# jskvrna/MonoSOWA

Hardware: AMD Instinct MI355X
Metric: MonoDETR training img/s (KITTI 1280x384) (higher is better)
Workload: dtype f32; 1 GPU; MonoDETR resnet50 KITTI 1280x384, fwd+criterion+bwd+AdamW step, per-GPU batch 16, synthetic images + random pseudo-labels; global_batch=16, per_gpu_batch=16, parallelism=dp1, accumulation_micro_steps=1, mixed_cameras=False, queries=550, tuned=True

## Files before the change

### monosowa_amd/csrc/msda_capi.hip

```cpp
#include "../../include/monosowa_msda.h"
#include "msda_kernels.hip"
#include "msda_backward_tiled.hip"
#include "msda_backward_sorted.hip"
#include "msda_backward_bands.hip"
#include "msda_gather_rec.hip"
#include "msda_gather_win.hip"
#include "msda_scatter_rows.hip"
#include "msda_plan.hip"
#include <map>
#include <mutex>
#include <cstdlib>
#include <string>
#include <algorithm>
#include <vector>

namespace {

inline int grid_for(long long work_items, int items_per_block) {
  long long g = (work_items + items_per_block - 1) / items_per_block;
  const long long cap = 256LL * 64;
  if (g > cap) g = cap;
  if (g < 1) g = 1;
  return (int)g;
}

inline int grid_pairs(long long n_pairs) { return (int)(((n_pairs + 31) / 32 + 7) / 8 * 8); }

inline int check_dims(int B, int S, int M, int D, int L, int Lq, int P) {
  if (B <= 0 || S <= 0 || M <= 0 || D <= 0 || L <= 0 || Lq <= 0 || P <= 0) return MSDA_E_SHAPE;
  if ((long long)S * M * D >= (1LL << 31)) return MSDA_E_SHAPE;
  if ((long long)B * Lq * M >= (1LL << 35)) return MSDA_E_SHAPE;
  return 0;
}

struct Options {
  int gather = 2;
  int scatter_fixed = 1;
  int scatter_sorted = 0;
  int gather_chunks_fwd = 16, gather_chunks_bwd = 8;
  int window = 3;
  int window_halo = 5;
  int window_persistent = 1;
  int scatter_rows = 1;
  int scatter_reach = 6;
  int directional = 1;
  int scatter_lists = 0;
  int scatter_lists_cap = 0;
  int scatter_bands = 1;
  int plan_fused = 1;
  int plan_reach = 8;
  int deterministic = 0;
  Options() {
    if (const char *e = std::getenv("MSDA_GATHER")) gather = std::atoi(e);
    if (const char *e = std::getenv("MSDA_SCATTER_FIXED")) scatter_fixed = std::atoi(e) != 0;
    if (const char *e = std::getenv("MSDA_SCATTER_SORTED")) scatter_sorted = std::atoi(e);
    if (const char *e = std::getenv("MSDA_GATHER_CHUNKS")) gather_chunks_fwd = std::max(1, std::atoi(e));
    if (const char *e = std::getenv("MSDA_GATHER_CHUNKS_BWD")) gather_chunks_bwd = std::max(1, std::atoi(e));
    if (const char *e = std::getenv("MSDA_WINDOW")) window = std::atoi(e) & 3;
    if (const char *e = std::getenv("MSDA_WINDOW_PERSISTENT")) window_persistent = std::atoi(e) != 0;
    if (const char *e = std::getenv("MSDA_SCATTER_ROWS")) scatter_rows = std::atoi(e) != 0;
    if (const char *e = std::getenv("MSDA_SCATTER_REACH")) scatter_reach = std::min(16, std::max(1, std::atoi(e)));
    if (const char *e = std::getenv("MSDA_WINDOW_HALO")) window_halo = std::min(32, std::max(0, std::atoi(e)));
    if (const char *e = std::getenv("MSDA_DIRECTIONAL")) directional = std::atoi(e) != 0;
    if (const char *e = std::getenv("MSDA_SCATTER_BANDS")) scatter_bands = std::atoi(e) != 0;
    if (const char *e = std::getenv("MSDA_SCATTER_LISTS")) scatter_lists = std::atoi(e) != 0;
    if (const char *e = std::getenv("MSDA_PLAN_FUSED")) plan_fused = std::atoi(e) != 0;
    if (const char *e = std::getenv("MSDA_PLAN_REACH")) plan_reach = std::min(16, std::max(1, std::atoi(e)));
  }
};
inline Options &options() {
  static Options o;
  return o;
}
inline bool scatter_fixed_point() { return options().scatter_fixed != 0; }
inline int gather_mode() { return options().gather; }
inline int gather_chunks_fwd() { return options().gather_chunks_fwd; }
inline int gather_chunks_bwd() { return options().gather_chunks_bwd; }

inline int check_host_geometry(const int64_t *shapes_host, const int64_t *lsi_host, int L, int S) {
  long long next = 0;
  for (int l = 0; l < L; ++l) {
    const long long H = shapes_host[2 * l], W = shapes_host[2 * l + 1];
    if (H <= 0 || W <= 0 || H > 32000 || W > 32000) return MSDA_E_SHAPE;
    if (lsi_host[l] != next) return MSDA_E_SHAPE;
    next += H * W;
  }
  return next == S ? 0 : MSDA_E_SHAPE;
}

bool make_gather_geom(const int64_t *shapes_host, const int64_t *lsi_host, int B, int M, int Lq, int S,
                      msda::GatherGeom &g, bool bwd = false) {
  int first = 4;
  long long rows = 0;
// ... 47 lines not shown
  static std::map<std::vector<int64_t>, msda::WinQuery *> cache;
  int dev = 0;
  if (hipGetDevice(&dev) != hipSuccess) return nullptr;
  std::vector<int64_t> key(shapes_host, shapes_host + 8);
  key.insert(key.end(), lsi_host, lsi_host + 4);
  key.push_back(halo);
  key.push_back(bwd);
  key.push_back(dev);
  std::lock_guard<std::mutex> lock(mu);
  auto it = cache.find(key);
  if (it == cache.end()) {
    std::vector<msda::WinQuery> host((size_t)wt.n_ty * wt.n_tx * msda::kWinMaxQueries * msda::kWinLevels);
    msda::fill_query_table(wt, host.data());
    msda::WinQuery *devp = nullptr;
    if (hipMalloc(&devp, host.size() * sizeof(msda::WinQuery)) != hipSuccess) return nullptr;
    if (hipMemcpy(devp, host.data(), host.size() * sizeof(msda::WinQuery), hipMemcpyHostToDevice) != hipSuccess) {
      (void)hipFree(devp);
      return nullptr;
    }
    it = cache.emplace(key, devp).first;
  }
  return it->second;
}

inline int persistent_grid() {
  static const int n = [] {
    int dev = 0, cus = 256;
    hipDeviceProp_t prop;
    if (hipGetDevice(&dev) == hipSuccess && hipGetDeviceProperties(&prop, dev) == hipSuccess && prop.multiProcessorCount > 0)
      cus = prop.multiProcessorCount;
    return std::max(8, cus / 8 * 8);
  }();
  return n;
}

constexpr int kWinMaxStride = 4096;
inline bool window_fits(int S, long long widest_stride) { return S < (1 << 17) && widest_stride <= kWinMaxStride; }

inline bool window_applies(bool bwd, const int64_t *shapes_host, const int64_t *lsi_host, int Lq, int S, long long widest_stride) {
  msda::WinGeom wg;
  return Lq == S && (options().window & (bwd ? 2 : 1)) && gather_mode() > 1 && window_fits(S, widest_stride) &&
         window_tiling(shapes_host, lsi_host, options().window_halo, bwd, wg);
}

thread_local int tl_launch_error = 0;
inline int launch_status() {
  const int e = tl_launch_error;
  tl_launch_error = 0;
  return e ? e : (int)hipGetLastError();
}

struct ValueView {
  int token_stride = 0;
  const unsigned char *mask = nullptr;
};

template <bool BWD, bool FUSED, bool SAVED = false>
void launch_gather(const float *value, const float *loc, const float *attw, const float *grad_out, float *out,
                   float *grad_loc, float *grad_attw, const float *ref, int ref_dim, const int64_t *shapes_host,
                   const int64_t *lsi_host, int B, int S, int M, int Lq, hipStream_t stream, int loc_rs = 0, int aw_rs = 0,
                   float *grad_value = nullptr, int far_reach = -1, ValueView vv = ValueView(),
                   const msda::HeadPlan *plans = nullptr, const unsigned char *far_mask = nullptr) {
  if (!loc_rs) loc_rs = M * 32;
  if (!aw_rs) aw_rs = M * 16;
  const int vts = vv.token_stride ? vv.token_stride : M * 32;
  if (Lq == S && (options().window & (BWD ? 2 : 1)) && gather_mode() > 1 && (!FUSED || ref_dim == 2)) {
// ... 170 lines not shown
            const int tiles = rp.n_ty[l] * rp.n_tx[l];
            bp.cap[l] = (int)std::min<long long>((3LL * Lq + tiles - 1) / tiles + 256, 16LL * msda::kRowChunkQueries);
            if (options().scatter_lists_cap > 0) bp.cap[l] = std::min(bp.cap[l], options().scatter_lists_cap);
            bp.list_off[l] = entries;
            n_tiles += tiles;
            entries += tiles * bp.cap[l];
            rp.n_chunks[l] = std::max(1, std::min(16, (bp.cap[l] + msda::kRowChunkQueries - 1) / msda::kRowChunkQueries));
            work[l] = (double)bp.cap[l] / rp.n_chunks[l];
            rp.order[l] = l;
          }
          bp.n_tiles = n_tiles; bp.plane_entries = entries;
          std::sort(rp.order, rp.order + 4, [&](int a, int b) { return work[a] > work[b]; });
          rp.first_item[0] = 0;
          for (int i = 0; i < 4; ++i) rp.first_item[i + 1] = rp.first_item[i] + rp.n_ty[rp.order[i]] * rp.n_tx[rp.order[i]] * rp.n_chunks[rp.order[i]];
          rp.n_items = rp.first_item[4];
          const size_t counts_b = align256(sizeof(unsigned) * (size_t)B * M * n_tiles);
          const size_t lists_b = align256(sizeof(unsigned) * (size_t)B * M * entries);
          const size_t far_b = align256((size_t)B * M * 4 * S);
          if ((long long)B * M * entries < (1LL << 31) && counts_b + lists_b + far_b <= workspace_bytes) {
            char *wsp = reinterpret_cast<char *>(workspace);
            unsigned *counts = reinterpret_cast<unsigned *>(wsp);
            unsigned *lists = reinterpret_cast<unsigned *>(wsp + counts_b);
            unsigned char *far_mask = reinterpret_cast<unsigned char *>(wsp + counts_b + lists_b);
            hipError_t e = hipMemsetAsync(counts, 0, counts_b, stream);
            if (e != hipSuccess) return (int)e;
            const long long n_units = (long long)B * M * 4 * S;
            msda::bin_points_kernel<<<(unsigned)((n_units + 255) / 256), 256, 0, stream>>>(loc, bp, n_units, S, counts, lists, far_mask);
            for (int l = 0; l < L; ++l) {
              if (rp.n_chunks[l] == 1) continue;
              e = hipMemset2DAsync(grad_value + (size_t)rp.start[l] * M * 32, sizeof(float) * (size_t)S * M * 32, 0,
                                   sizeof(float) * (size_t)rp.H[l] * rp.W[l] * M * 32, B, stream);
              if (e != hipSuccess) return (int)e;
            }
            const int groups = (B * M + 7) / 8;
            msda::scatter_rows_kernel<false, true><<<8 * rp.n_items * groups, msda::kRowThreads, 0, stream>>>(
                loc, attw, grad_out, grad_value, nullptr, 0, nullptr, rp, B, S, M, 0, 0, vv.mask, nullptr, lists, counts, bp, far_mask);
            launch_gather<true, true, true>(value, loc, attw, grad_out, nullptr, grad_loc, grad_attw, fused_ref, fused_ref_dim,
                                            shapes_host, lsi_host, B, S, M, Lq, stream, loc_rs, aw_rs, grad_value, 0, vv, nullptr, far_mask);
            return launch_status();
          }
        }
        bool directional = options().directional && (saved || fused_ref) && M <= msda::kPlanMaxHeads;
        int reach = 0;
        size_t plan_b = 0, stats_b = 0;
        bool ok = false;
        for (int attempt = 0; attempt < 2 && !ok; ++attempt) {
          reach = directional ? std::max(options().scatter_reach, options().plan_reach) : options().scatter_reach;
          plan_b = directional ? align256(msda::plan_bytes(M)) : 0;
          stats_b = directional ? align256(msda::plan_stats_bytes(M) * msda::kStatsBlocks) : 0;
          ok = msda::make_row_plan(shapes_host, lsi_host, reach, rp) && (!directional || rp.n_items <= msda::kPlanMaxItems) &&
               plan_b + stats_b + msda::row_plan_table_bytes(rp) * (directional ? M : 1) <= workspace_bytes;
          if (!ok) { if (!directional) break; directional = false; }
        }
        if (ok) {
          char *wsp = reinterpret_cast<char *>(workspace);
          msda::HeadPlan *plans = directional ? reinterpret_cast<msda::HeadPlan *>(wsp) : nullptr;
          msda::RowCandidate *table = reinterpret_cast<msda::RowCandidate *>(wsp + plan_b + stats_b);
          int n_tiles = 0;
          for (int l = 0; l < 4; ++l) n_tiles += rp.n_ty[l] * rp.n_tx[l];
          if (plan_mode && !(directional && saved)) return MSDA_E_UNSUPPORTED;
          if (directional && plan_mode != 2) {
            msda::PlanGeom pg{};
            for (int l = 0; l < 4; ++l) { pg.H[l] = rp.H[l]; pg.W[l] = rp.W[l]; pg.start[l] = rp.start[l]; }
            pg.S = S; pg.M = M;
            pg.default_halo = options().window_halo;
            pg.reach = reach;
            pg.want_rows = 1;
            if (options().plan_fused) {
              if (saved)
                msda::plan_fused_kernel<1><<<M * n_tiles, 256, 0, stream>>>(loc, nullptr, pg, rp, B, 0, n_tiles, plans, table);
              else
                msda::plan_fused_kernel<0><<<M * n_tiles, 256, 0, stream>>>(loc, fused_ref, pg, rp, B, loc_rs ? loc_rs : M * 32, n_tiles,
                                                                            plans, table);
            } else {
              msda::DirStats *partial = reinterpret_cast<msda::DirStats *>(wsp + plan_b);
              if (saved)
                msda::dir_stats_kernel<1><<<msda::kStatsBlocks, msda::kStatsThreads, 0, stream>>>(loc, nullptr, pg, B, 0, partial);
              else
                msda::dir_stats_kernel<0><<<msda::kStatsBlocks, msda::kStatsThreads, 0, stream>>>(
                    loc, fused_ref, pg, B, loc_rs ? loc_rs : M * 32, partial);
              msda::dir_plan_kernel<<<M, 256, 0, stream>>>(partial, msda::kStatsBlocks, pg, rp, plans);
            }
          }
          if (plan_mode != 2 && !(directional && options().plan_fused))
            msda::row_candidates_kernel<<<n_tiles * (directional ? M : 1), 256, 0, stream>>>(rp, table, plans, n_tiles);
          if (plan_mode == 1) return launch_status();
          for (int l = 0; l < L; ++l) {
            if (rp.n_chunks[l] == 1) continue;
            hipError_t e = hipMemset2DAsync(grad_value + (size_t)rp.start[l] * M * 32, sizeof(float) * (size_t)S * M * 32, 0,
                                            sizeof(float) * (size_t)rp.H[l] * rp.W[l] * M * 32, B, stream);
            if (e != hipSuccess) return (int)e;
          }
          const int groups = (B * M + 7) / 8;
          const int lrs = loc_rs ? loc_rs : M * 32, ars = aw_rs ? aw_rs : M * 16;
          if (fused_ref && !saved)
            msda::scatter_rows_kernel<true><<<8 * rp.n_items * groups, msda::kRowThreads, 0, stream>>>(
                loc, attw, grad_out, grad_value, fused_ref, fused_ref_dim, table, rp, B, S, M, lrs, ars, vv.mask, plans);
          else if (saved)
            msda::scatter_rows_kernel<false, true><<<8 * rp.n_items * groups, msda::kRowThreads, 0, stream>>>(
                loc, attw, grad_out, grad_value, nullptr, 0, table, rp, B, S, M, 0, 0, vv.mask, plans);
          else
            msda::scatter_rows_kernel<false><<<8 * rp.n_items * groups, msda::kRowThreads, 0, stream>>>(
                loc, attw, grad_out, grad_value, nullptr, 0, table, rp, B, S, M, lrs, ars);
          if (fused_ref && saved)
            launch_gather<true, true, true>(value, loc, attw, grad_out, nullptr, grad_loc, grad_attw, fused_ref, fused_ref_dim,
                                            shapes_host, lsi_host, B, S, M, Lq, stream, loc_rs, aw_rs, grad_value, rp.reach, vv, plans);
          else if (fused_ref)
            launch_gather<true, true>(value, loc, attw, grad_out, nullptr, grad_loc, grad_attw, fused_ref, fused_ref_dim,
                                      shapes_host, lsi_host, B, S, M, Lq, stream, loc_rs, aw_rs, grad_value, rp.reach, vv, plans);
          else
            launch_gather<true, false>(value, loc, attw, grad_out, nullptr, grad_loc, grad_attw, nullptr, 0, shapes_host,
                                       lsi_host, B, S, M, Lq, stream, 0, 0, grad_value, rp.reach);
          return launch_status();
        }
      }
      if (saved || plan_mode) return MSDA_E_UNSUPPORTED;
      const msda::BwdPlan plan = make_plan(shapes_host, lsi_host, L, Lq, P, det);
      if ((long long)Lq * P >= (1LL << (62 - msda::kFixBits))) return MSDA_E_SHAPE;
      const TiledWorkspace ws = tiled_workspace(B, M, L, Lq, P);
      char *wsp = reinterpret_cast<char *>(workspace);
      float2 *rec_hw = reinterpret_cast<float2 *>(wsp);
      float *rec_aw = reinterpret_cast<float *>(wsp + ws.off_aw);
      msda::ChunkBox *boxes = reinterpret_cast<msda::ChunkBox *>(wsp + ws.off_boxes);
      float *bounds = reinterpret_cast<float *>(wsp + ws.off_bounds);
      if (fused_ref)
        msda::bwd_prep_kernel<4, true><<<(unsigned)(B * ws.n_chunks_per_list), M * L * 8, 0, stream>>>(
            loc, attw, grad_out, shapes, rec_hw, rec_aw, boxes, fused_ref, fused_ref_dim, M, L, Lq, (int)ws.n_chunks_per_list,
            loc_rs ? loc_rs : M * 32, aw_rs ? aw_rs : M * 16);
      else
        msda::bwd_prep_kernel<4, false><<<(unsigned)(B * ws.n_chunks_per_list), M * L * 8, 0, stream>>>(
            loc, attw, grad_out, shapes, rec_hw, rec_aw, boxes, nullptr, 0, M, L, Lq, (int)ws.n_chunks_per_list, M * 32, M * 16);
      msda::BandPlan bp;
      const bool bands = !det && options().scatter_bands && options().scatter_sorted != 2 && L == 4 && P == 4 &&
                         msda::make_band_plan(shapes_host, lsi_host, Lq, bp);
      if (!bands) msda::bwd_bounds_kernel<<<B * M, 256, 0, stream>>>(boxes, bounds, (int)(L * ws.n_chunks_per_list));
      for (int l = 0; l < L && !bands; ++l) {
// ... 24 lines not shown
          launch_gather<true, false>(value, loc, attw, grad_out, nullptr, grad_loc, grad_attw, nullptr, 0, shapes_host,
                                     lsi_host, B, S, M, Lq, stream);
      } else {
        msda::bwd_gather_kernel<4, 4><<<grid_pairs(n_pairs), 256, 0, stream>>>(
            value, shapes, lsi, loc, attw, grad_out, grad_loc, grad_attw, S, M, Lq, n_pairs);
      }
      return launch_status();
    }
  }
  hipError_t err = hipMemsetAsync(grad_value, 0, sizeof(T) * (size_t)B * S * M * D, stream);
  if (err != hipSuccess) return (int)err;
  msda::bwd_generic_kernel<T><<<grid_for(n_pairs, 8), 256, 0, stream>>>(
      value, shapes, lsi, loc, attw, grad_out, grad_value, grad_loc, grad_attw, S, M, D, L, Lq, P,
      n_pairs);
  return launch_status();
}

}

extern "C" {

int msda_abi_version(void) { return MSDA_ABI_VERSION; }

int msda_set_option(const char *name, int value) {
  if (!name) return MSDA_E_NULLPTR;
  const std::string n(name);
  if (n == "gather" && value >= 0 && value <= 2) { options().gather = value; return 0; }
  if (n == "scatter_fixed" && (value == 0 || value == 1)) { options().scatter_fixed = value; return 0; }
  if (n == "scatter_sorted" && value >= 0 && value <= 2) { options().scatter_sorted = value; return 0; }
  if (n == "window" && value >= 0 && value <= 3) { options().window = value; return 0; }
  if (n == "window_halo" && value >= 0 && value <= 32) { options().window_halo = value; return 0; }
  if (n == "window_persistent" && (value == 0 || value == 1)) { options().window_persistent = value; return 0; }
  if (n == "scatter_rows" && (value == 0 || value == 1)) { options().scatter_rows = value; return 0; }
  if (n == "scatter_reach" && value >= 1 && value <= 16) { options().scatter_reach = value; return 0; }
  if (n == "directional" && (value == 0 || value == 1)) { options().directional = value; return 0; }
  if (n == "scatter_bands" && (value == 0 || value == 1)) { options().scatter_bands = value; return 0; }
  if (n == "scatter_lists" && (value == 0 || value == 1)) { options().scatter_lists = value; return 0; }
  if (n == "plan_reach" && value >= 1 && value <= 16) { options().plan_reach = value; return 0; }
  if (n == "plan_fused" && (value == 0 || value == 1)) { options().plan_fused = value; return 0; }
  if (n == "scatter_lists_cap" && value >= 0) { options().scatter_lists_cap = value; return 0; }
  if (n == "deterministic" && (value == 0 || value == 1)) { options().deterministic = value; return 0; }
  return MSDA_E_UNSUPPORTED;
}

int msda_options_stamp(void) {
  const Options &o = options();
  unsigned h = 2166136261u;
  for (int v : {o.directional, o.scatter_lists, o.scatter_rows, o.scatter_reach, o.plan_reach, o.plan_fused, o.window, o.window_halo, o.gather, o.deterministic}) {
    h ^= (unsigned)v + 0x9E3779B9u;
    h *= 16777619u;
  }
  return (int)(h & 0x7FFFFFFFu);
}

int msda_debug_counter(const char *name, unsigned long long *out) {
  if (!name || !out) return MSDA_E_NULLPTR;
  const std::string n(name);
  static const char *const scan_names[5] = {"scan_candidates", "scan_delivering", "scan_point_tests", "scan_delivered", "scan_points_skipped"};
  int scan = -1;
  for (int i = 0; i < 5; ++i)
    if (n == scan_names[i]) scan = i;
  if (n != "scatter_overflow_rounds" && scan < 0) return MSDA_E_UNSUPPORTED;
  const unsigned long long zero = 0;
  hipError_t e = hipDeviceSynchronize();
  if (scan >= 0) {
    if (e == hipSuccess) e = hipMemcpyFromSymbol(out, HIP_SYMBOL(msda::g_rows_scan), sizeof(zero), scan * sizeof(zero));
    if (e == hipSuccess) e = hipMemcpyToSymbol(HIP_SYMBOL(msda::g_rows_scan), &zero, sizeof(zero), scan * sizeof(zero));
    return (int)e;
  }
  if (e == hipSuccess) e = hipMemcpyFromSymbol(out, HIP_SYMBOL(msda::g_rows_overflow_rounds), sizeof(zero));
  if (e == hipSuccess) e = hipMemcpyToSymbol(HIP_SYMBOL(msda::g_rows_overflow_rounds), &zero, sizeof(zero));
  return (int)e;
}

const char *msda_strerror(int code) {
  switch (code) {
    case 0: return "success";
    case MSDA_E_NULLPTR: return "msda: a required pointer is NULL";
    case MSDA_E_SHAPE: return "msda: a dimension is <= 0 or exceeds the indexing range";
    case MSDA_E_UNSUPPORTED: return "msda: unsupported configuration";
    case MSDA_E_WORKSPACE: return "msda: workspace is NULL or smaller than msda_backward_workspace_bytes()";
// ... 261 lines not shown
```

### monosowa_amd/csrc/msda_scatter_rows.hip

```cpp
#include "msda_common.h"
#include "msda_scatter_plan.h"
#include "msda_plan.h"
#include "msda_bin.hip"

#ifndef MSDA_ROWS_SKIP
#define MSDA_ROWS_SKIP 0
#endif
#ifndef MSDA_ROWS_STAMP
#define MSDA_ROWS_STAMP 0
#endif

namespace msda {

#if MSDA_ROWS_STAMP
__device__ unsigned long long g_rows_stamp[8];
#define ROWS_STAMP(i) do { const long long t_ = clock64(); st_acc[i] += t_ - st_t; st_t = t_; } while (0)
#else
#define ROWS_STAMP(i) do { } while (0)
#endif

typedef float rows_v2f __attribute__((ext_vector_type(2)));

__device__ unsigned long long g_rows_overflow_rounds;

#ifndef MSDA_ROWS_PRIO
#define MSDA_ROWS_PRIO 0
#endif
#ifndef MSDA_ROWS_COUNT
#define MSDA_ROWS_COUNT 0
#endif
__device__ unsigned long long g_rows_scan[5];

__device__ __forceinline__ void lds_barrier() {
  asm volatile("s_waitcnt lgkmcnt(0)\n\ts_barrier" ::: "memory");
}

__global__ __launch_bounds__(256) void row_candidates_kernel(const RowPlan p, RowCandidate *__restrict__ table,
                                                             const HeadPlan *__restrict__ plans, int n_tiles) {
  const int head = blockIdx.x / n_tiles;
  int l = 0, t = blockIdx.x - head * n_tiles;
  while (l < 3 && t >= p.n_ty[l] * p.n_tx[l]) { t -= p.n_ty[l] * p.n_tx[l]; ++l; }
  const int ty = t / p.n_tx[l], tx = t - ty * p.n_tx[l];
  const RowAxis *axes = plans ? plans[head].rax : p.ax;
  const RowAxis ay = axes[p.axis0[l] + ty], ax = axes[p.axis0[l] + p.n_ty[l] + tx];
  RowCandidate *out = table + (long long)head * p.cand_total + p.cand_base[l] + (long long)t * p.cand_stride[l];
  int first = 0;
  for (int lq = 0; lq < 4; ++lq) {
    const int n = (int)ay.qn[lq] * (int)ax.qn[lq], w = ax.qn[lq];
    for (int k = threadIdx.x; k < n; k += 256) {
      const int dy = k / w, dx = k - dy * w;
      const int yq = ay.q0[lq] + dy, xq = ax.q0[lq] + dx;
      RowCandidate c;
      c.token = p.start[lq] + yq * p.W[lq] + xq;
      c.cy = (short)centre_floor(yq, p.H[lq], p.H[l]);
      c.cx = (short)centre_floor(xq, p.W[lq], p.W[l]);
      out[first + k] = c;
    }
    first += n;
  }
}

#ifndef MSDA_ROW_WAVES
#define MSDA_ROW_WAVES 4
#endif
template <bool FUSED, bool LEVEL_MAJOR = false>
__global__ __launch_bounds__(kRowThreads, MSDA_ROW_WAVES) void scatter_rows_kernel(
    const float *__restrict__ loc, const float *__restrict__ attw, const float *__restrict__ grad_out,
    float *__restrict__ grad_value, const float *__restrict__ ref, int ref_dim, const RowCandidate *__restrict__ table,
    const RowPlan p, int B, int S, int M, int loc_rs, int aw_rs, const unsigned char *__restrict__ vmask = nullptr,
    const HeadPlan *__restrict__ plans = nullptr, const unsigned *__restrict__ lists = nullptr,
    const unsigned *__restrict__ counts = nullptr, const BinPlan bp = BinPlan(),
    const unsigned char *__restrict__ far_mask = nullptr) {
  __shared__ float4 lds_pool[kRowBatchQueries * 8 + kRowBatchQueries * 4];
  float4 *const go_lds = lds_pool;
  float4 *const coef_tab = lds_pool + kRowBatchQueries * 8;
  static_assert(kRowThreads * 6 <= kRowBatchQueries * 12, "the epilogue's exchange fits the pool");
  __shared__ unsigned short bucket[kRowTileRows * (kRowCellCap + 1)];
  __shared__ unsigned count[kRowTileRows];
  __shared__ int overflow;

  const int bm = (int)(blockIdx.x % 8) + 8 * (int)(blockIdx.x / (8 * p.n_items));
  if (bm >= B * M) return;
  const int it = (int)((blockIdx.x / 8) % p.n_items);
  const int b = bm / M, m = bm - b * M;
  const HeadPlan *hp = plans ? plans + m : nullptr;
  int l, n_chunks, y0, th, x0, tw, c_begin, c_end;
  const RowCandidate *cands;
  DirBounds nb;
  bool by_list = false;
  const unsigned *list = nullptr;
  if (lists) {
    int oi = 0;
    while (oi < 3 && it >= p.first_item[oi + 1]) ++oi;
    l = p.order[oi];
    const int local = it - p.first_item[oi];
    n_chunks = p.n_chunks[l];
    const int chunk = local % n_chunks, tile = local / n_chunks;
    const int ty = tile / p.n_tx[l], tx = tile - ty * p.n_tx[l];
    const RowAxis ay = p.ax[p.axis0[l] + ty], ax = p.ax[p.axis0[l] + p.n_ty[l] + tx];
    y0 = ay.r0; x0 = ax.r0; th = ay.rn; tw = ax.rn;
    const int n_list = (int)min(counts[(long long)bm * bp.n_tiles + bp.tile0[l] + tile], (unsigned)bp.cap[l]);
    c_begin = chunk * kRowChunkQueries;
    c_end = min(n_list, c_begin + kRowChunkQueries);
    if (c_end <= c_begin) {
      if (chunk > 0) return;
      c_end = c_begin;
    }
    list = lists + (long long)bm * bp.plane_entries + bp.list_off[l] + (long long)tile * bp.cap[l];
    cands = nullptr;
    nb.ylo = nb.xlo = nb.yhi = nb.xhi = 0;
    by_list = true;
  } else if (hp) {
    if (it >= hp->n_items) return;
    const RowItem d = hp->items[it];
    l = d.level; n_chunks = d.n_chunks;
    y0 = d.y0; th = d.th; x0 = d.x0; tw = d.tw;
    c_begin = d.c_begin; c_end = d.c_end;
    cands = table + (long long)m * p.cand_total + d.cand_off;
    nb = d.near;
  } else {
    int oi = 0;
    while (oi < 3 && it >= p.first_item[oi + 1]) ++oi;
    l = p.order[oi];
    const int local = it - p.first_item[oi];
    n_chunks = p.n_chunks[l];
    const int chunk = local % n_chunks, tile = local / n_chunks;
    const int ty = tile / p.n_tx[l], tx = tile - ty * p.n_tx[l];
    const RowAxis ay = p.ax[p.axis0[l] + ty], ax = p.ax[p.axis0[l] + p.n_ty[l] + tx];
    nb.ylo = nb.xlo = (short)-p.reach; nb.yhi = nb.xhi = (short)p.reach;
    y0 = ay.r0; x0 = ax.r0; th = ay.rn; tw = ax.rn;
    int n_cand = 0;
#pragma unroll
    for (int lq = 0; lq < 4; ++lq) n_cand += (int)ay.qn[lq] * (int)ax.qn[lq];
    c_begin = (int)((long long)n_cand * chunk / n_chunks);
    c_end = (int)((long long)n_cand * (chunk + 1) / n_chunks);
    cands = table + p.cand_base[l] + (long long)tile * p.cand_stride[l];
  }
  const int H = p.H[l], W = p.W[l];
  const int cw = tw + 1, n_cells = (th + 1) * cw;
  constexpr int cap = kRowCellCap, bstride = kRowCellCap + 1;

  const int tid = threadIdx.x;
  const int slot0 = tid >> 2, pt = tid & 3;
  const int cell = tid >> 2, quarter = tid & 3;
  if (tid < kRowTileRows) count[tid] = 0;
  if (tid == 0) overflow = 0;
  rows_v2f sums[4][4];
#pragma unroll
  for (int j = 0; j < 4; ++j)
#pragma unroll
    for (int i = 0; i < 4; ++i) sums[j][i] = (rows_v2f){0.f, 0.f};

  struct Points { float4 lg; float2 xy; float wt; RefScale rs; };
  const int n_batches = (MSDA_ROWS_SKIP & 128) ? 1 : (c_end - c_begin + kRowBatchQueries - 1) / kRowBatchQueries;
  auto cand_index = [&](const int k, const int u) {
    return k < n_batches ? c_begin + k + (slot0 + u * (kRowThreads / 4)) * n_batches : c_end;
  };
  auto candidate = [&](const int j) {
    RowCandidate c{-1, 0, 0};
    if (j < c_end) {
      if (by_list) {
        const unsigned e = list[j];
        c.token = (int)(e & 0x0FFFFFFFu);
        c.cy = (short)((e >> 28) & ~(unsigned)far_mask[((long long)bm * 4 + l) * S + c.token]);
      } else {
        c = cands[j];
      }
    }
    return c;
  };
#if MSDA_ROWS_COUNT
  unsigned n_scan[5] = {0, 0, 0, 0, 0};
#endif
  auto fetch = [&](const RowCandidate c) {
    Points in{};
    if (c.token >= 0) {
      const long long q_lin = (long long)b * S + c.token;
      const long long pl = (((long long)(b * M + m) * 4 + l) * S + c.token) * 4 + pt;
      in.xy = LEVEL_MAJOR ? *reinterpret_cast<const float2 *>(loc + pl * 2)
                          : *reinterpret_cast<const float2 *>(loc + q_lin * loc_rs + ((m * 4 + l) * 4 + pt) * 2);
      if (FUSED) {
        const float *lg = attw + q_lin * aw_rs + m * 16;
        in.lg = ld4(lg + pt * 4);
        in.wt = lg[l * 4 + pt];
        in.rs = load_ref(ref + (q_lin * 4 + l) * ref_dim, ref_dim, H, W);
      } else {
        in.wt = LEVEL_MAJOR ? attw[pl] : attw[q_lin * aw_rs + (m * 4 + l) * 4 + pt];
      }
    }
    return in;
  };
  RowCandidate cur[kRowSub], c_next[kRowSub];
  Points in[kRowSub];
#pragma unroll
  for (int u = 0; u < kRowSub; ++u) {
    cur[u] = candidate(cand_index(0, u));
    in[u] = fetch(cur[u]);
    c_next[u] = candidate(cand_index(1, u));
  }
  lds_barrier();
#if MSDA_ROWS_STAMP
  long long st_acc[8] = {0, 0, 0, 0, 0, 0, 0, 0}, st_t = clock64();
#endif

  for (int k = 0; k < n_batches; ++k) {
    ROWS_STAMP(0);
#if MSDA_ROWS_PRIO == 1
    __builtin_amdgcn_s_setprio(2);
#elif MSDA_ROWS_PRIO == 2
    __builtin_amdgcn_s_setprio(0);
#endif
    float4 g0[kRowSub], g1[kRowSub];
#pragma unroll
    for (int u = 0; u < kRowSub; ++u) {
      g0[u] = g1[u] = make_float4(0.f, 0.f, 0.f, 0.f);
      if (cur[u].token >= 0 && !(MSDA_ROWS_SKIP & 16)) {
        const float *gp = grad_out + (((long long)b * S + cur[u].token) * M + m) * 32 + pt * 8;
        g0[u] = ld4(gp);
        g1[u] = ld4(gp + 4);
      }
    }
    unsigned pend = 0;
    int cells[kRowSub];
#pragma unroll
    for (int u = 0; u < kRowSub; ++u) {
      const int slot = slot0 + u * (kRowThreads / 4);
      float lx = in[u].xy.x, ly = in[u].xy.y, wt = in[u].wt;
      if (FUSED) {
        const float4 lg = in[u].lg;
        float mx = fmaxf(fmaxf(lg.x, lg.y), fmaxf(lg.z, lg.w));
        mx = fmaxf(mx, dpp_x<0xB1>(mx)); mx = fmaxf(mx, dpp_x<0x4E>(mx));
        float sum = expf(lg.x - mx) + expf(lg.y - mx) + expf(lg.z - mx) + expf(lg.w - mx);
        sum += dpp_x<0xB1>(sum); sum += dpp_x<0x4E>(sum);
        wt = expf(wt - mx) / sum;
        lx = loc_from_offset<4>(in[u].rs.rx, lx, in[u].rs.sx, ref_dim);
        ly = loc_from_offset<4>(in[u].rs.ry, ly, in[u].rs.sy, ref_dim);
      }
      cells[u] = 0;
      if (cur[u].token >= 0 && (!(MSDA_ROWS_SKIP & 32) || lx == 123.456f)) {
#if MSDA_ROWS_COUNT
        n_scan[0] += pt == 0;
        ++n_scan[2];
#endif
        const Tap<float> tp = make_tap<float>(lx, ly, H, W);
        if (tp.valid && (by_list ? (cur[u].cy >> pt & 1) != 0 : inside_bounds(tp.h_low - cur[u].cy, tp.w_low - cur[u].cx, nb))) {
          const int cy = tp.h_low - (y0 - 1), cx = tp.w_low - (x0 - 1);
          if ((unsigned)cy <= (unsigned)th && (unsigned)cx <= (unsigned)tw) {
            cells[u] = cy * cw + cx;
            coef_tab[slot * 4 + pt] = make_float4(tp.w1 * wt, tp.w2 * wt, tp.w3 * wt, tp.w4 * wt);
            if (!(MSDA_ROWS_SKIP & 2)) pend |= 1u << u;
          }
        }
      }
    }
#pragma unroll
    for (int u = 0; u < kRowSub; ++u) {
      unsigned any = (pend >> u) & 1u;
#if MSDA_ROWS_COUNT
      n_scan[3] += any;
#endif
      any |= (unsigned)__builtin_amdgcn_update_dpp(0, (int)any, 0xB1, 0xF, 0xF, false);
      any |= (unsigned)__builtin_amdgcn_update_dpp(0, (int)any, 0x4E, 0xF, 0xF, false);
#if MSDA_ROWS_COUNT
      n_scan[1] += any && pt == 0;
#endif
      if (any) {
        const int slot = slot0 + u * (kRowThreads / 4);
        go_lds[slot * 8 + ((pt * 2) ^ (slot & 7))] = g0[u];
        go_lds[slot * 8 + ((pt * 2 + 1) ^ (slot & 7))] = g1[u];
      }
      cur[u] = c_next[u];
      in[u] = fetch(cur[u]);
      c_next[u] = candidate(cand_index(k + 2, u));
    }
    ROWS_STAMP(1);
#if MSDA_ROWS_PRIO == 1
    __builtin_amdgcn_s_setprio(0);
#elif MSDA_ROWS_PRIO == 2
    __builtin_amdgcn_s_setprio(2);
#endif
    bool again;
    do {
      unsigned rank[kRowSub];
#pragma unroll
      for (int u = 0; u < kRowSub; ++u) {
        rank[u] = 0xFFFFFFFFu;
        if (pend & (1u << u)) rank[u] = atomicAdd(&count[cells[u]], 1u);
      }
#pragma unroll
      for (int u = 0; u < kRowSub; ++u)
        if (rank[u] < (unsigned)cap) {
          bucket[cells[u] * bstride + rank[u]] = (unsigned short)((slot0 + u * (kRowThreads / 4)) * 4 + pt);
          pend &= ~(1u << u);
        }
      if (pend) overflow = 1;
      ROWS_STAMP(2);
      lds_barrier();
      ROWS_STAMP(3);
      again = overflow != 0;
      if (cell < n_cells) {
        const int n = min((int)count[cell], cap);
        const unsigned short *bk = bucket + cell * bstride;
        const char *go_b = reinterpret_cast<const char *>(go_lds);
        const int hs = quarter << 5;
        unsigned idx_next = bk[0];
        for (int i = 0; i < ((MSDA_ROWS_SKIP & 1) ? 0 : n); ++i) {
          const unsigned idx = idx_next;
          idx_next = bk[i + 1];
          const float4 c4 = coef_tab[idx];
          const unsigned s4 = idx >> 2, a0 = ((s4 << 7) | ((s4 & 7) << 4)) ^ hs;
          float4 a[2];
#pragma unroll
          for (int kk = 0; kk < 2; ++kk) a[kk] = *reinterpret_cast<const float4 *>(go_b + (a0 ^ (kk << 4)));
#pragma unroll
          for (int kk = 0; kk < 2; ++kk) {
            const rows_v2f lo = (rows_v2f){a[kk].x, a[kk].y}, hi = (rows_v2f){a[kk].z, a[kk].w};
            sums[0][2 * kk] = __builtin_elementwise_fma((rows_v2f){c4.x, c4.x}, lo, sums[0][2 * kk]);
            sums[0][2 * kk + 1] = __builtin_elementwise_fma((rows_v2f){c4.x, c4.x}, hi, sums[0][2 * kk + 1]);
            sums[1][2 * kk] = __builtin_elementwise_fma((rows_v2f){c4.y, c4.y}, lo, sums[1][2 * kk]);
            sums[1][2 * kk + 1] = __builtin_elementwise_fma((rows_v2f){c4.y, c4.y}, hi, sums[1][2 * kk + 1]);
            sums[2][2 * kk] = __builtin_elementwise_fma((rows_v2f){c4.z, c4.z}, lo, sums[2][2 * kk]);
            sums[2][2 * kk + 1] = __builtin_elementwise_fma((rows_v2f){c4.z, c4.z}, hi, sums[2][2 * kk + 1]);
            sums[3][2 * kk] = __builtin_elementwise_fma((rows_v2f){c4.w, c4.w}, lo, sums[3][2 * kk]);
            sums[3][2 * kk + 1] = __builtin_elementwise_fma((rows_v2f){c4.w, c4.w}, hi, sums[3][2 * kk + 1]);
          }
        }
        if (quarter == 0) count[cell] = 0;
      }
      ROWS_STAMP(4);
      lds_barrier();
      ROWS_STAMP(5);
      if (again) {
        if (tid == 0) { overflow = 0; atomicAdd(&g_rows_overflow_rounds, 1ull); }
        lds_barrier();
      }
    } while (again);
  }

#if MSDA_ROWS_COUNT
  for (int i = 0; i < 5; ++i) {
    unsigned v = n_scan[i];
    for (int o = 32; o > 0; o >>= 1) v += __shfl_xor(v, o);
    if ((threadIdx.x & 63) == 0 && v) atomicAdd(&g_rows_scan[i], (unsigned long long)v);
  }
#endif
#if MSDA_ROWS_STAMP
  ROWS_STAMP(6);
  if ((threadIdx.x & 63) == 0)
    for (int i = 0; i < 8; ++i) atomicAdd(&g_rows_stamp[i], (unsigned long long)st_acc[i]);
#endif
  if ((MSDA_ROWS_SKIP & 64) && sums[0][0].x != 123.456f) return;
  const int cy = cell / cw, cx = cell - cy * cw;
  const bool is_out = cell < n_cells && cy >= 1 && cx >= 1;
  {
    float4 *mine = lds_pool + (cell * 4 + quarter) * 6;
#pragma unroll
    for (int j = 1; j < 4; ++j)
#pragma unroll
      for (int kk = 0; kk < 2; ++kk)
        mine[(j - 1) * 2 + kk] = make_float4(sums[j][2 * kk].x, sums[j][2 * kk].y, sums[j][2 * kk + 1].x, sums[j][2 * kk + 1].y);
    lds_barrier();
    if (is_out) {
      const int src[3] = {cell - 1, cell - cw, cell - cw - 1};
#pragma unroll
      for (int j = 0; j < 3; ++j)
#pragma unroll
        for (int kk = 0; kk < 2; ++kk) {
          const float4 v = lds_pool[(src[j] * 4 + quarter) * 6 + j * 2 + kk];
          sums[0][2 * kk] += (rows_v2f){v.x, v.y};
          sums[0][2 * kk + 1] += (rows_v2f){v.z, v.w};
        }
    }
  }

  float4 acc[2];
#pragma unroll
  for (int k = 0; k < 2; ++k) acc[k] = make_float4(sums[0][2 * k].x, sums[0][2 * k].y, sums[0][2 * k + 1].x, sums[0][2 * k + 1].y);
  const long long tok0 = (long long)b * S + p.start[l];
  if (n_chunks == 1) {
    if (is_out) {
      const long long token = tok0 + (long long)(y0 + cy - 1) * W + (x0 + cx - 1);
      float *dst = grad_value + (token * M + m) * 32 + quarter * 8;
      const bool padded = vmask && vmask[token];
#pragma unroll
      for (int k = 0; k < 2; ++k) st4(dst + 4 * k, padded ? make_float4(0.f, 0.f, 0.f, 0.f) : acc[k]);
    }
  } else {
    lds_barrier();
    float *rows_lds = reinterpret_cast<float *>(go_lds);
    if (is_out) {
#pragma unroll
      for (int k = 0; k < 2; ++k) *reinterpret_cast<float4 *>(rows_lds + cell * 32 + quarter * 8 + 4 * k) = acc[k];
    }
    __syncthreads();
    const int ch = tid & 31;
    for (int rr = tid >> 5; rr < n_cells; rr += kRowThreads / 32) {
      const int ry = rr / cw, rx = rr - ry * cw;
      if (ry < 1 || rx < 1) continue;
      const float v = rows_lds[rr * 32 + ch];
      const long long token = tok0 + (long long)(y0 + ry - 1) * W + (x0 + rx - 1);
      if (v != 0.f && !(vmask && vmask[token])) atomicAdd(grad_value + (token * M + m) * 32 + ch, v);
    }
  }
}

}
```

Before: 248.0 img/s.

## Add optional persistent work-loop to scatter_rows kernel with cross-item prefetch

Restructures the row-scatter backward kernel so each workgroup can loop over several plan items, assigned round-robin in a serpentine order. The next item's descriptor is decoded and its first candidates prefetched while the current item is processed, through scalar constant-address loads. Persistence is off by default (scatter_persistent=0), so each workgroup still handles exactly one item. The default path nonetheless runs the rewritten loop, which adds register pressure and extra barrier and selection logic.

```diff
diff --git a/monosowa_amd/csrc/msda_capi.hip b/monosowa_amd/csrc/msda_capi.hip
--- a/monosowa_amd/csrc/msda_capi.hip
+++ b/monosowa_amd/csrc/msda_capi.hip
@@ -42,6 +42,8 @@
   int window_halo = 5;
   int window_persistent = 1;
   int scatter_rows = 1;
+  int scatter_persistent = 0;
+  int scatter_persistent_wgs = 0;
   int scatter_reach = 6;
   int directional = 1;
   int scatter_lists = 0;
@@ -59,6 +61,7 @@
     if (const char *e = std::getenv("MSDA_WINDOW")) window = std::atoi(e) & 3;
     if (const char *e = std::getenv("MSDA_WINDOW_PERSISTENT")) window_persistent = std::atoi(e) != 0;
     if (const char *e = std::getenv("MSDA_SCATTER_ROWS")) scatter_rows = std::atoi(e) != 0;
+    if (const char *e = std::getenv("MSDA_SCATTER_PERSISTENT")) scatter_persistent = std::atoi(e) != 0;
     if (const char *e = std::getenv("MSDA_SCATTER_REACH")) scatter_reach = std::min(16, std::max(1, std::atoi(e)));
     if (const char *e = std::getenv("MSDA_WINDOW_HALO")) window_halo = std::min(32, std::max(0, std::atoi(e)));
     if (const char *e = std::getenv("MSDA_DIRECTIONAL")) directional = std::atoi(e) != 0;
@@ -172,6 +175,13 @@
     return std::max(8, cus / 8 * 8);
   }();
   return n;
+}
+
+inline int scatter_rows_wgs(int n_items, int groups) {
+  const Options &o = options();
+  if (!o.scatter_persistent) return n_items;
+  const int w = o.scatter_persistent_wgs > 0 ? o.scatter_persistent_wgs : 2 * persistent_grid() / (8 * groups);
+  return std::max(1, std::min(w, n_items));
 }
 
 constexpr int kWinMaxStride = 4096;
@@ -408,9 +418,9 @@
                                    sizeof(float) * (size_t)rp.H[l] * rp.W[l] * M * 32, B, stream);
               if (e != hipSuccess) return (int)e;
             }
-            const int groups = (B * M + 7) / 8;
-            msda::scatter_rows_kernel<false, true><<<8 * rp.n_items * groups, msda::kRowThreads, 0, stream>>>(
-                loc, attw, grad_out, grad_value, nullptr, 0, nullptr, rp, B, S, M, 0, 0, vv.mask, nullptr, lists, counts, bp, far_mask);
+            const int groups = (B * M + 7) / 8, wgs = scatter_rows_wgs(rp.n_items, groups);
+            msda::scatter_rows_kernel<false, true><<<8 * wgs * groups, msda::kRowThreads, 0, stream>>>(
+                loc, attw, grad_out, grad_value, nullptr, 0, nullptr, rp, B, S, M, 0, 0, wgs, vv.mask, nullptr, lists, counts, bp, far_mask);
             launch_gather<true, true, true>(value, loc, attw, grad_out, nullptr, grad_loc, grad_attw, fused_ref, fused_ref_dim,
                                             shapes_host, lsi_host, B, S, M, Lq, stream, loc_rs, aw_rs, grad_value, 0, vv, nullptr, far_mask);
             return launch_status();
@@ -467,17 +477,17 @@
                                             sizeof(float) * (size_t)rp.H[l] * rp.W[l] * M * 32, B, stream);
             if (e != hipSuccess) return (int)e;
           }
-          const int groups = (B * M + 7) / 8;
+          const int groups = (B * M + 7) / 8, wgs = scatter_rows_wgs(rp.n_items, groups);
           const int lrs = loc_rs ? loc_rs : M * 32, ars = aw_rs ? aw_rs : M * 16;
           if (fused_ref && !saved)
-            msda::scatter_rows_kernel<true><<<8 * rp.n_items * groups, msda::kRowThreads, 0, stream>>>(
-                loc, attw, grad_out, grad_value, fused_ref, fused_ref_dim, table, rp, B, S, M, lrs, ars, vv.mask, plans);
+            msda::scatter_rows_kernel<true><<<8 * wgs * groups, msda::kRowThreads, 0, stream>>>(
+                loc, attw, grad_out, grad_value, fused_ref, fused_ref_dim, table, rp, B, S, M, lrs, ars, wgs, vv.mask, plans);
           else if (saved)
-            msda::scatter_rows_kernel<false, true><<<8 * rp.n_items * groups, msda::kRowThreads, 0, stream>>>(
-                loc, attw, grad_out, grad_value, nullptr, 0, table, rp, B, S, M, 0, 0, vv.mask, plans);
+            msda::scatter_rows_kernel<false, true><<<8 * wgs * groups, msda::kRowThreads, 0, stream>>>(
+                loc, attw, grad_out, grad_value, nullptr, 0, table, rp, B, S, M, 0, 0, wgs, vv.mask, plans);
           else
-            msda::scatter_rows_kernel<false><<<8 * rp.n_items * groups, msda::kRowThreads, 0, stream>>>(
-                loc, attw, grad_out, grad_value, nullptr, 0, table, rp, B, S, M, lrs, ars);
+            msda::scatter_rows_kernel<false><<<8 * wgs * groups, msda::kRowThreads, 0, stream>>>(
+                loc, attw, grad_out, grad_value, nullptr, 0, table, rp, B, S, M, lrs, ars, wgs);
           if (fused_ref && saved)
             launch_gather<true, true, true>(value, loc, attw, grad_out, nullptr, grad_loc, grad_attw, fused_ref, fused_ref_dim,
                                             shapes_host, lsi_host, B, S, M, Lq, stream, loc_rs, aw_rs, grad_value, rp.reach, vv, plans);
@@ -568,6 +578,8 @@
   if (n == "window_halo" && value >= 0 && value <= 32) { options().window_halo = value; return 0; }
   if (n == "window_persistent" && (value == 0 || value == 1)) { options().window_persistent = value; return 0; }
   if (n == "scatter_rows" && (value == 0 || value == 1)) { options().scatter_rows = value; return 0; }
+  if (n == "scatter_persistent" && (value == 0 || value == 1)) { options().scatter_persistent = value; return 0; }
+  if (n == "scatter_persistent_wgs" && value >= 0 && value <= 4096) { options().scatter_persistent_wgs = value; return 0; }
   if (n == "scatter_reach" && value >= 1 && value <= 16) { options().scatter_reach = value; return 0; }
   if (n == "directional" && (value == 0 || value == 1)) { options().directional = value; return 0; }
   if (n == "scatter_bands" && (value == 0 || value == 1)) { options().scatter_bands = value; return 0; }
@@ -582,7 +594,8 @@
 int msda_options_stamp(void) {
   const Options &o = options();
   unsigned h = 2166136261u;
-  for (int v : {o.directional, o.scatter_lists, o.scatter_rows, o.scatter_reach, o.plan_reach, o.plan_fused, o.window, o.window_halo, o.gather, o.deterministic}) {
+  for (int v : {o.directional, o.scatter_lists, o.scatter_rows, o.scatter_reach, o.plan_reach, o.plan_fused, o.window, o.window_halo, o.gather, o.deterministic,
+                o.scatter_persistent, o.scatter_persistent_wgs}) {
     h ^= (unsigned)v + 0x9E3779B9u;
     h *= 16777619u;
   }
diff --git a/monosowa_amd/csrc/msda_scatter_rows.hip b/monosowa_amd/csrc/msda_scatter_rows.hip
--- a/monosowa_amd/csrc/msda_scatter_rows.hip
+++ b/monosowa_amd/csrc/msda_scatter_rows.hip
@@ -33,6 +33,11 @@
 
 __device__ __forceinline__ void lds_barrier() {
   asm volatile("s_waitcnt lgkmcnt(0)\n\ts_barrier" ::: "memory");
+}
+
+__device__ __forceinline__ int uniform_ld(const void *base, const int i) {
+  typedef const __attribute__((address_space(4))) int *const_int_p;
+  return ((const_int_p)(unsigned long long)base)[i];
 }
 
 __global__ __launch_bounds__(256) void row_candidates_kernel(const RowPlan p, RowCandidate *__restrict__ table,
@@ -67,7 +72,7 @@
 __global__ __launch_bounds__(kRowThreads, MSDA_ROW_WAVES) void scatter_rows_kernel(
     const float *__restrict__ loc, const float *__restrict__ attw, const float *__restrict__ grad_out,
     float *__restrict__ grad_value, const float *__restrict__ ref, int ref_dim, const RowCandidate *__restrict__ table,
-    const RowPlan p, int B, int S, int M, int loc_rs, int aw_rs, const unsigned char *__restrict__ vmask = nullptr,
+    const RowPlan p, int B, int S, int M, int loc_rs, int aw_rs, int wgs, const unsigned char *__restrict__ vmask = nullptr,
     const HeadPlan *__restrict__ plans = nullptr, const unsigned *__restrict__ lists = nullptr,
     const unsigned *__restrict__ counts = nullptr, const BinPlan bp = BinPlan(),
     const unsigned char *__restrict__ far_mask = nullptr) {
@@ -79,65 +84,67 @@
   __shared__ unsigned count[kRowTileRows];
   __shared__ int overflow;
 
-  const int bm = (int)(blockIdx.x % 8) + 8 * (int)(blockIdx.x / (8 * p.n_items));
+  const int bm = (int)(blockIdx.x % 8) + 8 * (int)(blockIdx.x / (8 * wgs));
   if (bm >= B * M) return;
-  const int it = (int)((blockIdx.x / 8) % p.n_items);
+  const int w_id = (int)((blockIdx.x / 8) % wgs);
   const int b = bm / M, m = bm - b * M;
   const HeadPlan *hp = plans ? plans + m : nullptr;
-  int l, n_chunks, y0, th, x0, tw, c_begin, c_end;
-  const RowCandidate *cands;
-  DirBounds nb;
-  bool by_list = false;
-  const unsigned *list = nullptr;
-  if (lists) {
-    int oi = 0;
-    while (oi < 3 && it >= p.first_item[oi + 1]) ++oi;
-    l = p.order[oi];
-    const int local = it - p.first_item[oi];
-    n_chunks = p.n_chunks[l];
-    const int chunk = local % n_chunks, tile = local / n_chunks;
-    const int ty = tile / p.n_tx[l], tx = tile - ty * p.n_tx[l];
-    const RowAxis ay = p.ax[p.axis0[l] + ty], ax = p.ax[p.axis0[l] + p.n_ty[l] + tx];
-    y0 = ay.r0; x0 = ax.r0; th = ay.rn; tw = ax.rn;
-    const int n_list = (int)min(counts[(long long)bm * bp.n_tiles + bp.tile0[l] + tile], (unsigned)bp.cap[l]);
-    c_begin = chunk * kRowChunkQueries;
-    c_end = min(n_list, c_begin + kRowChunkQueries);
-    if (c_end <= c_begin) {
-      if (chunk > 0) return;
-      c_end = c_begin;
-    }
-    list = lists + (long long)bm * bp.plane_entries + bp.list_off[l] + (long long)tile * bp.cap[l];
-    cands = nullptr;
-    nb.ylo = nb.xlo = nb.yhi = nb.xhi = 0;
-    by_list = true;
-  } else if (hp) {
-    if (it >= hp->n_items) return;
-    const RowItem d = hp->items[it];
-    l = d.level; n_chunks = d.n_chunks;
-    y0 = d.y0; th = d.th; x0 = d.x0; tw = d.tw;
-    c_begin = d.c_begin; c_end = d.c_end;
-    cands = table + (long long)m * p.cand_total + d.cand_off;
-    nb = d.near;
-  } else {
-    int oi = 0;
-    while (oi < 3 && it >= p.first_item[oi + 1]) ++oi;
-    l = p.order[oi];
-    const int local = it - p.first_item[oi];
-    n_chunks = p.n_chunks[l];
-    const int chunk = local % n_chunks, tile = local / n_chunks;
-    const int ty = tile / p.n_tx[l], tx = tile - ty * p.n_tx[l];
-    const RowAxis ay = p.ax[p.axis0[l] + ty], ax = p.ax[p.axis0[l] + p.n_ty[l] + tx];
-    nb.ylo = nb.xlo = (short)-p.reach; nb.yhi = nb.xhi = (short)p.reach;
-    y0 = ay.r0; x0 = ax.r0; th = ay.rn; tw = ax.rn;
-    int n_cand = 0;
-#pragma unroll
-    for (int lq = 0; lq < 4; ++lq) n_cand += (int)ay.qn[lq] * (int)ax.qn[lq];
-    c_begin = (int)((long long)n_cand * chunk / n_chunks);
-    c_end = (int)((long long)n_cand * (chunk + 1) / n_chunks);
-    cands = table + p.cand_base[l] + (long long)tile * p.cand_stride[l];
-  }
-  const int H = p.H[l], W = p.W[l];
-  const int cw = tw + 1, n_cells = (th + 1) * cw;
+  const bool by_list = lists != nullptr;
+  struct Item {
+    int state;
+    int l, n_chunks;
+    int yt, xt;
+    int c_begin, c_end, n_batches;
+    int nby, nbx;
+    const void *src;
+  };
+  auto pair16 = [](const int lo, const int hi) { return (lo & 0xFFFF) | (hi << 16); };
+  auto item_of_round = [&](const int r) { return r * wgs + ((r & 1) ? wgs - 1 - w_id : w_id); };
+  auto decode = [&](const int it) {
+    Item d{};
+    if (it >= p.n_items) return d;
+    if (hp && !by_list) {
+      const void *r = hp->items + it;
+      const int lc = uniform_ld(r, 0), nc = uniform_ld(r, 1), cand_off = uniform_ld(r, 6);
+      d.yt = uniform_ld(r, 2); d.xt = uniform_ld(r, 3);
+      d.c_begin = uniform_ld(r, 4); d.c_end = uniform_ld(r, 5);
+      d.nby = uniform_ld(r, 8); d.nbx = uniform_ld(r, 9);
+      if (it >= uniform_ld(&hp->n_items, 0)) return d;
+      d.l = (short)lc; d.n_chunks = (short)nc;
+      d.src = table + (long long)m * p.cand_total + cand_off;
+    } else {
+      int oi = 0;
+      while (oi < 3 && it >= p.first_item[oi + 1]) ++oi;
+      d.l = p.order[oi];
+      const int local = it - p.first_item[oi];
+      d.n_chunks = p.n_chunks[d.l];
+      const int chunk = local % d.n_chunks, tile = local / d.n_chunks;
+      const int ty = tile / p.n_tx[d.l], tx = tile - ty * p.n_tx[d.l];
+      const RowAxis ay = p.ax[p.axis0[d.l] + ty], ax = p.ax[p.axis0[d.l] + p.n_ty[d.l] + tx];
+      d.yt = pair16(ay.r0, ay.rn); d.xt = pair16(ax.r0, ax.rn);
+      if (by_list) {
+        const int n_list = (int)min((unsigned)uniform_ld(counts + ((long long)bm * bp.n_tiles + bp.tile0[d.l] + tile), 0), (unsigned)bp.cap[d.l]);
+        d.c_begin = chunk * kRowChunkQueries;
+        d.c_end = min(n_list, d.c_begin + kRowChunkQueries);
+        if (d.c_end <= d.c_begin) {
+          if (chunk > 0) { d.state = 2; return d; }
+          d.c_end = d.c_begin;
+        }
+        d.src = lists + (long long)bm * bp.plane_entries + bp.list_off[d.l] + (long long)tile * bp.cap[d.l];
+      } else {
+        d.nby = d.nbx = pair16(-p.reach, p.reach);
+        int n_cand = 0;
+#pragma unroll
+        for (int lq = 0; lq < 4; ++lq) n_cand += (int)ay.qn[lq] * (int)ax.qn[lq];
+        d.c_begin = (int)((long long)n_cand * chunk / d.n_chunks);
+        d.c_end = (int)((long long)n_cand * (chunk + 1) / d.n_chunks);
+        d.src = table + p.cand_base[d.l] + (long long)tile * p.cand_stride[d.l];
+      }
+    }
+    d.n_batches = (MSDA_ROWS_SKIP & 128) ? 1 : (d.c_end - d.c_begin + kRowBatchQueries - 1) / kRowBatchQueries;
+    d.state = 1;
+    return d;
+  };
   constexpr int cap = kRowCellCap, bstride = kRowCellCap + 1;
 
   const int tid = threadIdx.x;
@@ -145,26 +152,27 @@
   const int cell = tid >> 2, quarter = tid & 3;
   if (tid < kRowTileRows) count[tid] = 0;
   if (tid == 0) overflow = 0;
-  rows_v2f sums[4][4];
-#pragma unroll
-  for (int j = 0; j < 4; ++j)
-#pragma unroll
-    for (int i = 0; i < 4; ++i) sums[j][i] = (rows_v2f){0.f, 0.f};
 
   struct Points { float4 lg; float2 xy; float wt; RefScale rs; };
-  const int n_batches = (MSDA_ROWS_SKIP & 128) ? 1 : (c_end - c_begin + kRowBatchQueries - 1) / kRowBatchQueries;
-  auto cand_index = [&](const int k, const int u) {
-    return k < n_batches ? c_begin + k + (slot0 + u * (kRowThreads / 4)) * n_batches : c_end;
-  };
-  auto candidate = [&](const int j) {
-    RowCandidate c{-1, 0, 0};
-    if (j < c_end) {
+  struct Cand { int token, yx; };
+  static_assert(sizeof(RowCandidate) == 8, "a candidate entry is read as two dwords");
+  Item A{}, N{};
+  auto candidate = [&](const int f, const int u) {
+    const bool own = f < A.n_batches;
+    const int k = own ? f : f - A.n_batches;
+    const int nb_i = own ? A.n_batches : N.n_batches, l_i = own ? A.l : N.l;
+    const int cb = own ? A.c_begin : N.c_begin, ce = own ? A.c_end : N.c_end;
+    const void *src = own ? A.src : N.src;
+    Cand c{-1, 0};
+    const int j = cb + k + (slot0 + u * (kRowThreads / 4)) * nb_i;
+    if (k < nb_i && j < ce) {
       if (by_list) {
-        const unsigned e = list[j];
+        const unsigned e = static_cast<const unsigned *>(src)[j];
         c.token = (int)(e & 0x0FFFFFFFu);
-        c.cy = (short)((e >> 28) & ~(unsigned)far_mask[((long long)bm * 4 + l) * S + c.token]);
+        c.yx = (int)((e >> 28) & ~(unsigned)far_mask[((long long)bm * 4 + l_i) * S + c.token]);
       } else {
-        c = cands[j];
+        const int2 e = static_cast<const int2 *>(src)[j];
+        c.token = e.x; c.yx = e.y;
       }
     }
     return c;
@@ -172,9 +180,11 @@
 #if MSDA_ROWS_COUNT
   unsigned n_scan[5] = {0, 0, 0, 0, 0};
 #endif
-  auto fetch = [&](const RowCandidate c) {
+  unsigned n_again = 0;
+  auto fetch = [&](const Cand c, const int f) {
     Points in{};
     if (c.token >= 0) {
+      const int l = f < A.n_batches ? A.l : N.l;
       const long long q_lin = (long long)b * S + c.token;
       const long long pl = (((long long)(b * M + m) * 4 + l) * S + c.token) * 4 + pt;
       in.xy = LEVEL_MAJOR ? *reinterpret_cast<const float2 *>(loc + pl * 2)
@@ -183,25 +193,53 @@
         const float *lg = attw + q_lin * aw_rs + m * 16;
         in.lg = ld4(lg + pt * 4);
         in.wt = lg[l * 4 + pt];
-        in.rs = load_ref(ref + (q_lin * 4 + l) * ref_dim, ref_dim, H, W);
+        in.rs = load_ref(ref + (q_lin * 4 + l) * ref_dim, ref_dim, p.H[l], p.W[l]);
       } else {
         in.wt = LEVEL_MAJOR ? attw[pl] : attw[q_lin * aw_rs + (m * 4 + l) * 4 + pt];
       }
     }
     return in;
   };
-  RowCandidate cur[kRowSub], c_next[kRowSub];
+  Cand cur[kRowSub], c_next[kRowSub];
   Points in[kRowSub];
 #pragma unroll
-  for (int u = 0; u < kRowSub; ++u) {
-    cur[u] = candidate(cand_index(0, u));
-    in[u] = fetch(cur[u]);
-    c_next[u] = candidate(cand_index(1, u));
-  }
-  lds_barrier();
+  for (int u = 0; u < kRowSub; ++u) { cur[u] = c_next[u] = Cand{-1, 0}; in[u] = Points{}; }
 #if MSDA_ROWS_STAMP
   long long st_acc[8] = {0, 0, 0, 0, 0, 0, 0, 0}, st_t = clock64();
 #endif
+
+  for (int step = 0, round = 0;; ++step) {
+  if (step > 1) {
+    if (N.state == 0) break;
+    lds_barrier();
+  }
+  A = N;
+  do N = decode(item_of_round(round++)); while (N.state == 2);
+  if (step == 0) continue;
+  if (A.state == 0) break;
+  if (step == 1 || A.n_batches < 2) {
+#pragma unroll
+    for (int u = 0; u < kRowSub; ++u) {
+      if (step == 1 || A.n_batches == 0) {
+        cur[u] = candidate(0, u);
+        in[u] = fetch(cur[u], 0);
+      }
+      c_next[u] = candidate(1, u);
+    }
+  }
+  if (step == 1) lds_barrier();
+  ROWS_STAMP(7);
+  const int l = A.l, n_chunks = A.n_chunks, n_batches = A.n_batches;
+  const int y0 = (short)A.yt, th = A.yt >> 16, x0 = (short)A.xt, tw = A.xt >> 16;
+  DirBounds nb;
+  nb.ylo = (short)A.nby; nb.yhi = (short)(A.nby >> 16); nb.xlo = (short)A.nbx; nb.xhi = (short)(A.nbx >> 16);
+  const int H = p.H[l], W = p.W[l];
+  const int cw = tw + 1, n_cells = (th + 1) * cw;
+  rows_v2f sums[4][4];
+#pragma unroll
+  for (int j = 0; j < 4; ++j)
+#pragma unroll
+    for (int i = 0; i < 4; ++i) sums[j][i] = (rows_v2f){0.f, 0.f};
 
   for (int k = 0; k < n_batches; ++k) {
     ROWS_STAMP(0);
@@ -243,7 +281,7 @@
         ++n_scan[2];
 #endif
         const Tap<float> tp = make_tap<float>(lx, ly, H, W);
-        if (tp.valid && (by_list ? (cur[u].cy >> pt & 1) != 0 : inside_bounds(tp.h_low - cur[u].cy, tp.w_low - cur[u].cx, nb))) {
+        if (tp.valid && (by_list ? (cur[u].yx >> pt & 1) != 0 : inside_bounds(tp.h_low - (short)cur[u].yx, tp.w_low - (cur[u].yx >> 16), nb))) {
           const int cy = tp.h_low - (y0 - 1), cx = tp.w_low - (x0 - 1);
           if ((unsigned)cy <= (unsigned)th && (unsigned)cx <= (unsigned)tw) {
             cells[u] = cy * cw + cx;
@@ -269,9 +307,12 @@
         go_lds[slot * 8 + ((pt * 2) ^ (slot & 7))] = g0[u];
         go_lds[slot * 8 + ((pt * 2 + 1) ^ (slot & 7))] = g1[u];
       }
+    }
+#pragma unroll
+    for (int u = 0; u < kRowSub; ++u) {
       cur[u] = c_next[u];
-      in[u] = fetch(cur[u]);
-      c_next[u] = candidate(cand_index(k + 2, u));
+      in[u] = fetch(cur[u], k + 1);
+      c_next[u] = candidate(k + 2, u);
     }
     ROWS_STAMP(1);
 #if MSDA_ROWS_PRIO == 1
@@ -331,25 +372,15 @@
       lds_barrier();
       ROWS_STAMP(5);
       if (again) {
-        if (tid == 0) { overflow = 0; atomicAdd(&g_rows_overflow_rounds, 1ull); }
+        if (tid == 0) overflow = 0;
+        ++n_again;
         lds_barrier();
       }
     } while (again);
   }
 
-#if MSDA_ROWS_COUNT
-  for (int i = 0; i < 5; ++i) {
-    unsigned v = n_scan[i];
-    for (int o = 32; o > 0; o >>= 1) v += __shfl_xor(v, o);
-    if ((threadIdx.x & 63) == 0 && v) atomicAdd(&g_rows_scan[i], (unsigned long long)v);
-  }
-#endif
-#if MSDA_ROWS_STAMP
   ROWS_STAMP(6);
-  if ((threadIdx.x & 63) == 0)
-    for (int i = 0; i < 8; ++i) atomicAdd(&g_rows_stamp[i], (unsigned long long)st_acc[i]);
-#endif
-  if ((MSDA_ROWS_SKIP & 64) && sums[0][0].x != 123.456f) return;
+  if (!((MSDA_ROWS_SKIP & 64) && sums[0][0].x != 123.456f)) {
   const int cy = cell / cw, cx = cell - cy * cw;
   const bool is_out = cell < n_cells && cy >= 1 && cx >= 1;
   {
@@ -392,7 +423,7 @@
 #pragma unroll
       for (int k = 0; k < 2; ++k) *reinterpret_cast<float4 *>(rows_lds + cell * 32 + quarter * 8 + 4 * k) = acc[k];
     }
-    __syncthreads();
+    lds_barrier();
     const int ch = tid & 31;
     for (int rr = tid >> 5; rr < n_cells; rr += kRowThreads / 32) {
       const int ry = rr / cw, rx = rr - ry * cw;
@@ -402,6 +433,22 @@
       if (v != 0.f && !(vmask && vmask[token])) atomicAdd(grad_value + (token * M + m) * 32 + ch, v);
     }
   }
+  }
+  }
+
+  if (tid == 0 && n_again) atomicAdd(&g_rows_overflow_rounds, (unsigned long long)n_again);
+#if MSDA_ROWS_COUNT
+  for (int i = 0; i < 5; ++i) {
+    unsigned v = n_scan[i];
+    for (int o = 32; o > 0; o >>= 1) v += __shfl_xor(v, o);
+    if ((threadIdx.x & 63) == 0 && v) atomicAdd(&g_rows_scan[i], (unsigned long long)v);
+  }
+#endif
+#if MSDA_ROWS_STAMP
+  ROWS_STAMP(7);
+  if ((threadIdx.x & 63) == 0)
+    for (int i = 0; i < 8; ++i) atomicAdd(&g_rows_stamp[i], (unsigned long long)st_acc[i]);
+#endif
 }
 
 }
```

Measured after the change: 242.4 img/s. -2.3%, worse.
